# brontoguana/krasis

Measured on AMD Instinct MI355X. Metric: decode tok/s, Qwen3-Coder-Next Q4 @1 MI355X (KR_DECODE_FAST tolerance mode; both modes: value_exact / value_fast), higher is better.
Workload: dtype int4-g128 w x int16 act -> i32, f32 scales; 1 GPU; Qwen3-Coder-Next Q4 int4gpu on 1×MI355X (512-expert top-10, hybrid linear+GQA, FP8 KV); kv=FP8-E4M3 KV cache, kv_max_seq 256, layers=48, parallelism=one GPU holds the whole model (N > 1 lines: expert parallelism, see main_multi), hip_graph=True

## Files before the change

krasis_amd/csrc/kr_decode.cpp:

```cpp
#include <algorithm>
#include <hip/hip_runtime.h>

#include <cmath>
#include <cstring>
#include <memory>
#include <string>
#include <vector>

#include "../../include/krasis_hip.h"
#include "kr_decode_ops.h"
#include "kr_engine_internal.h"
#include "kr_kernels.h"
#include "kr_prefill.h"
#include "kr_router.h"
#include "kr_sampler.h"
#include <chrono>

#include "kr_decode_internal.h"
#include "kr_decode_fast.h"

static void prof_mark(kr_decode_store* s, int kind, hipStream_t st) {
    if (!s->prof) return;
    if (s->ev_used + 2 > s->ev_pool.size()) { for (int i = 0; i < 64; i++) { hipEvent_t e; (void)hipEventCreate(&e); s->ev_pool.push_back(e); } }
    if (kind >= 0) s->ev_kind.push_back(kind);
// ... 626 lines not shown
    PROF(PK_MATVEC, kr_launch_matvec(mv(s, L.mqb_wid), s->proj_b.p, 1, q_full, st));
}

static int attn_mla(StepCtx& cx, DLayer& L, size_t li) {
    kr_decode_store* s = cx.s; hipStream_t st = cx.st;
    if (!L.kv_k.p) return kr_fail(KR_ERR_STATE, "set_decode_state was not called (no MLA cache for layer %zu)", li);
    if (L.mla_rope_seq < s->kv_max_seq) return kr_fail(KR_ERR_VALUE, "MLA rope table (%d) shorter than kv_max_seq (%d)", L.mla_rope_seq, s->kv_max_seq);
    float* kv_out = (float*)s->kbuf.p; float* q_full = (float*)s->proj_a.p;
    const bool lora = L.mq_wid < 0;
    if (!cx.did_in) {
        const int wids[2] = {L.kva_wid, lora ? L.mqa_wid : L.mq_wid};
        float* ys[2] = {kv_out, lora ? (float*)s->proj_b.p : q_full};
        proj_group(cx, wids, ys, 2, cx.hid, 1);
    }
    if (lora) mla_lora_tail(cx, L, q_full);
    KrMlaArgs a{};
    a.step = (const KrStep*)s->step_dev.p; a.kv_out = kv_out; a.q_full = q_full; a.kv_a_norm = (const float*)L.kv_a_norm.p; a.w_kc = (const float*)L.w_kc.p;
    a.w_vc = (const float*)L.w_vc.p; a.rope_cos = (const float*)L.mla_cos.p; a.rope_sin = (const float*)L.mla_sin.p;
    a.ckv_cache = L.kv_k.p; a.kpe_cache = L.kv_v.p; a.kv_fp8 = s->kv_fp8; a.q_abs = (float*)s->qbuf.p; a.q_pe = (float*)s->zbuf.p;
    a.attn_lat = (float*)s->latbuf.p; a.v_proj = (float*)s->attn_out.p;
    a.nh = L.nh; a.klr = L.klr; a.nd = L.nd; a.rd = L.rd; a.vhd = L.vhd; a.eps = s->eps; a.sm_scale = L.sm_scale;
    a.sc_g = s->kv_max_seq > s->mla_split_min ? (float*)s->gqa_scores.p : nullptr;
    if (s->attn_fast && a.sc_g) { a.fast = 1; a.fd_o = (float*)s->fd_o.p; a.fd_ml = (float*)s->fd_ml.p; }
    a.decode_fast = cx.fast ? 1 : 0; a.decode_fused = cx.fast && s->opt_gqa_fused ? 1 : 0;
    PROF(PK_GQA, kr_launch_mla(a, s->kv_max_seq, st));
    if (cx.fast && s->weights[L.o_wid]->cols == L.nh * L.vhd) {
        KrFdmArgs fo = fdm_one(s, 2, L.o_wid, cx.hid); fo.hid_in = (const float*)s->attn_out.p;
        if (PROF_RC(PK_OUT_PROJ, kr_launch_fdm(fo, st)) == 0) return KR_OK;
    }
    out_proj(cx, L.o_wid, false);
    return KR_OK;
}

static int fast_moe(StepCtx& cx, DLayer& L, Layer& EL, size_t li, bool* done) {
    kr_decode_store* s = cx.s; kr_engine* e = cx.e; hipStream_t st = cx.st;
    if (EL.gguf && cx.src.mode == 2) return KR_OK;
    const MoeShape m = moe_shape(s, L, EL);
    KrFmoeArgs fa{}; KrMoeArgs& a = fa.m;
    moe_args_common(cx, L, m, a);
    a.act_img = s->img_post.p; a.act_img_bf16 = s->img_post_bf16.p;
    a.ids = (const int32_t*)s->r_ids.p; a.wts = (const float*)s->r_w.p;
    a.topk = s->topk; a.n_slots = m.n_slots; a.I = EL.inter; a.gu = (float*)s->moe_gu.p; a.eo = (float*)s->moe_eo.p;
    bool ok = true;
    if (EL.gguf) {
        fa.gguf = 1; fa.ggate = EL.g_gate.view(); fa.gup = EL.g_up.view(); fa.gdown = EL.g_down.view(); fa.act_f32 = (const float*)s->hid2.p;
        a.E = e->cfg.n_routed_experts; ok = e->r_ne == e->cfg.n_routed_experts;
    } else { a.E = e->r_ne; a.w13 = EL.w13.view(); a.w2 = EL.w2.view(); }
    if (m.has_gate) {
        const KrMatDev sg = mv(s, L.sg_wid);
        if (EL.gguf ? sg.bits == a.sw13.bits : (a.w13.bits == a.sw13.bits && sg.bits == a.w13.bits)) { a.sgate = sg; a.gate_out = (float*)s->gate_val.p; }
        else ok = false;
    }
    fa.logits = (const float*)s->r_logits.p; fa.esc = route_esc(EL); fa.scoring = s->scoring; fa.norm_topk = s->norm_topk;
    fa.hid_out = cx.hid;
    if (cx.ep_dec) {
        kr_ep_slice(e, &a.e_lo, &a.e_hi, &a.e_sub);
        fa.shared_skip = m.has_shared && kr_ep_rank(e) != (int)(li % (size_t)kr_ep_world(e)) ? 1 : 0;
    }
    if (!ok || kr_fmoe_check(fa) != 0) return KR_OK;
    if (PROF_RC(PK_ROUTE_LOGITS, kr_launch_frt(frt_args(cx, L, EL), st)) != 0) return KR_OK;
    const int r13 = PROF_RC(PK_MOE_W13, kr_launch_fw13(fa, st));
    const int r2 = PROF_RC(PK_MOE_W2, kr_launch_fw2(fa, st));
    if ((r13 || r2) && EL.gguf) return kr_fail(KR_ERR_STATE, "internal: KR_DECODE_FAST expert launch refused after kr_fmoe_check accepted GGUF layer %zu", li);
    if (r13 || r2) return kr_fail(KR_ERR_STATE, "internal: KR_DECODE_FAST expert launch refused after kr_fmoe_check accepted layer %zu", li);
    if (cx.ep_dec) if (int rc = kr_ep_allreduce_on(e, cx.hid, (size_t)cx.H, st)) return rc;
    cx.res_cur = cx.other(); cx.src = KrNormSrc{}; *done = true;
    return KR_OK;
}

static bool dense_fast(StepCtx& cx, DLayer& L) {
    kr_decode_store* s = cx.s; hipStream_t st = cx.st;
    const KrMatDev g = mv(s, L.gate_wid), u = mv(s, L.up_wid);
    const int K = s->weights[L.down_wid]->cols;
    if (!(g.bits == u.bits && (g.bits == 4 || g.bits == 8))) return false;
    KrFdmArgs fd = fdm_one(s, 1, L.gate_wid, (float*)s->dense_gu.p);
    fdm_norm(cx, L.post_norm, fd);
    fd.mm.n = 2; fd.mm.m[1] = u; fd.mm.y[1] = (float*)s->dense_gu.p + K; fd.mm.tile_end[1] = fd.mm.tile_end[0] + (u.N + 7) / 8;
    if (PROF_RC(PK_MATVEC, kr_launch_fdm(fd, st)) != 0) return false;
    cx.res_cur = cx.other();
    PROF(PK_MATVEC, kr_launch_matvec(mv(s, L.down_wid), s->dense_gu.p, 1, cx.hid, st, KR_ACT_SILU_MUL));
    return true;
}

static int moe_exact_gguf(StepCtx& cx, DLayer& L, Layer& EL, const float* act, bool routed) {
    kr_decode_store* s = cx.s; kr_engine* e = cx.e; hipStream_t st = cx.st;
    const MoeShape m = moe_shape(s, L, EL);
    const int k = s->topk, H = cx.H;
    GgMoeArgs g{};
    g.B = 1; g.topk = k; g.n_slots = k; g.H = H; g.E = e->cfg.n_routed_experts; g.act_f32 = act; g.ids = (const int32_t*)s->r_ids.p;
    g.gate = EL.g_gate.view(); g.up = EL.g_up.view(); g.down = EL.g_down.view();
    g.I_max = EL.inter; g.gu_ld = 2 * m.imax;
    g.gu = (float*)s->moe_gu.p; g.eo = (float*)s->moe_eo.p;
    PROF(PK_MOE_W13, kr_launch_gguf_moe(g, st));
    if (m.has_shared) {
        KrMoeArgs a{};
        moe_args_common(cx, L, m, a);
        a.act_f32 = act; if (routed && cx.img_ok()) { a.act_img = s->img_post.p; a.act_img_bf16 = s->img_post_bf16.p; }
        a.topk = 0; a.n_slots = 1; a.E = 0; a.I = m.I_shared;
        a.w13 = a.sw13; a.w2 = a.sw2;
        a.gu = g.gu + (size_t)k * g.gu_ld; a.eo = g.eo + (size_t)k * H;
        const bool fuse_gate = m.has_gate && mv(s, L.sg_wid).bits == a.sw13.bits;
        if (fuse_gate) { a.sgate = mv(s, L.sg_wid); a.gate_out = (float*)s->gate_val.p; }
        PROF(PK_MOE_W13, kr_launch_moe_w13(a, st));
        if (m.has_gate && !fuse_gate) PROF(PK_SHARED_GATE, kr_launch_matvec(mv(s, L.sg_wid), act, 1, (float*)s->gate_val.p, st));
        PROF(PK_MOE_W2, kr_launch_moe_w2(a, st));
    }
    if (cx.fast) {
// ... 159 lines not shown
    if (token == KR_TOKEN_FROM_DEVICE) kr_launch_set_step_dev((KrStep*)s->step_dev.p, (const int*)s->tok.p, pos, st);
    else kr_launch_set_step((KrStep*)s->step_dev.p, token, pos, st);
    s->last_stream = st;
    const bool ep_active = kr_ep_decode_active(s->eng);
    if (s->eng->ep_generation != s->ep_generation_seen) {
        s->ep_generation_seen = s->eng->ep_generation; s->graph_ok = false; s->ep_eager_steps = 0;
    }
    if (ep_active && s->ep_eager_steps < 2) s->ep_eager_steps++;
    else if (s->use_graph && (!ep_active || (s->opt_ep_graph && kr_ep_is_rccl(s->eng)))) {
        if (!s->graph_ok) {
            if (s->graph_exec) { (void)hipGraphExecDestroy(s->graph_exec); s->graph_exec = nullptr; }
            hipGraph_t g = nullptr;
            KR_HIP(hipStreamBeginCapture(st, hipStreamCaptureModeThreadLocal));
            const int rc = enqueue_step(s, st);
            hipError_t ce = hipStreamEndCapture(st, &g);
            if (rc) { if (g) (void)hipGraphDestroy(g); return rc; }
            if (ce != hipSuccess) return kr_fail(KR_ERR_HIP, "hipStreamEndCapture failed: %s", hipGetErrorString(ce));
            KR_HIP(hipGraphInstantiate(&s->graph_exec, g, nullptr, nullptr, 0));
            (void)hipGraphDestroy(g);
            s->graph_ok = true;
        }
        KR_HIP(hipGraphLaunch(s->graph_exec, st));
        return KR_OK;
    }
    return enqueue_step(s, st);
}

extern "C" int kr_decode_set_kv_dtype(kr_decode_store* s, int kv_dtype) {
    if (int rc = chk_store(s)) return rc;
    if (kv_dtype != 0 && kv_dtype != 1) return kr_fail(KR_ERR_VALUE, "kv_dtype %d unknown (0 = FP16, 1 = FP8-E4M3)", kv_dtype);
    if (s->kv_fp8 != kv_dtype) for (auto& L : s->layers) if (L.attn == ATTN_GQA || L.attn == ATTN_MLA) { L.kv_k.release(); L.kv_v.release(); }
    s->kv_fp8 = kv_dtype; s->graph_ok = false;
    return KR_OK;
}

extern "C" int kr_decode_set_attention_mode(kr_decode_store* s, int mode) {
    if (int rc = chk_store(s)) return rc;
    if (mode < 0 || mode > 7) return kr_fail(KR_ERR_VALUE, "numerics mode %d unknown (bit 0 = KR_ATTN_FAST, bit 1 = KR_GEMM_FAST, bit 2 = KR_DECODE_FAST)", mode);
    s->attn_fast = mode & 1; s->gemm_fast = (mode >> 1) & 1; s->decode_fast = (mode >> 2) & 1; s->graph_ok = false;
    return KR_OK;
}

extern "C" int kr_decode_set_option(kr_decode_store* s, const char* name, int value) {
    if (int rc = chk_store(s)) return rc;
    if (!name) return kr_fail(KR_ERR_VALUE, "null option name");
    if (!strcmp(name, "gqa_stream")) { s->opt_gqa_stream = value != 0; s->graph_ok = false; return KR_OK; }
    if (!strcmp(name, "w2_combine")) { s->opt_w2_combine = value != 0; s->graph_ok = false; return KR_OK; }
    if (!strcmp(name, "la_heads")) { s->opt_la_heads = value != 0; s->graph_ok = false; return KR_OK; }
    if (!strcmp(name, "lm_fused")) { s->opt_lm_fused = value != 0; s->graph_ok = false; return KR_OK; }
    if (!strcmp(name, "gqa_fused")) { s->opt_gqa_fused = value != 0; s->graph_ok = false; return KR_OK; }
    if (!strcmp(name, "gemm_ring")) { kr_pfr_set_enabled(value); return KR_OK; }
    if (!strcmp(name, "la_conv_fused")) { s->opt_la_conv_fused = value != 0; return KR_OK; }
    if (!strcmp(name, "dense_fast")) { s->opt_dense_fast = value != 0; s->graph_ok = false; return KR_OK; }
    if (!strcmp(name, "norm_rows")) { s->opt_norm_rows = value != 0; return KR_OK; }
    if (!strcmp(name, "pfm_timing")) { s->opt_pfm_timing = value != 0; return KR_OK; }
    if (!strcmp(name, "generate_lookahead")) { s->opt_gen_lookahead = value != 0; return KR_OK; }
    if (!strcmp(name, "multi_sample_loop")) { s->opt_multi_sample_loop = value != 0; return KR_OK; }
    if (!strcmp(name, "multi_attn_fast")) { s->opt_multi_attn_fast = value != 0; return KR_OK; }
    if (!strcmp(name, "multi_attn_fast_paged")) { s->opt_multi_attn_fast_paged = value != 0; return KR_OK; }
    if (!strcmp(name, "multi_mla_fast")) { s->opt_multi_mla_fast = value != 0; return KR_OK; }
    if (!strcmp(name, "multi_extend_la_chunk")) { s->opt_multi_extend_la_chunk = value != 0; return KR_OK; }
    if (!strcmp(name, "multi_extend_exact_mfma")) { s->opt_multi_extend_exact_mfma = value != 0; return KR_OK; }
    if (!strcmp(name, "multi_extend_mla_exact_mfma")) { s->opt_multi_extend_mla_exact_mfma = value != 0; return KR_OK; }
    if (!strcmp(name, "multi_attn_exact_split")) { s->opt_multi_attn_exact_split = value != 0; return KR_OK; }
    if (!strcmp(name, "multi_attn_exact_split_min")) {
        if (value < 1) return kr_fail(KR_ERR_VALUE, "multi_attn_exact_split_min %d: at least 1", value);
        s->opt_multi_attn_exact_split_min = value; return KR_OK;
    }
    if (!strcmp(name, "multi_mla_exact_split")) { s->opt_multi_mla_exact_split = value != 0; return KR_OK; }
    if (!strcmp(name, "multi_mla_exact_split_min")) {
        if (value < 1) return kr_fail(KR_ERR_VALUE, "multi_mla_exact_split_min %d: at least 1", value);
        s->opt_multi_mla_exact_split_min = value; return KR_OK;
    }
    if (!strcmp(name, "multi_extend_flash")) { s->opt_multi_extend_flash = value != 0; return KR_OK; }
    if (!strcmp(name, "multi_extend_mla_flash")) { s->opt_multi_extend_mla_flash = value != 0; return KR_OK; }
    if (!strcmp(name, "gguf_exact_pass")) { s->opt_gguf_exact_pass = value != 0; return KR_OK; }
    if (!strcmp(name, "gguf_exact_grouped")) { s->opt_gguf_exact_grouped = value != 0; return KR_OK; }
    if (!strcmp(name, "ep_graph")) { s->opt_ep_graph = value != 0; s->graph_ok = false; return KR_OK; }
    return kr_fail(KR_ERR_VALUE, "unknown option '%s'", name);
}

extern "C" int kr_decode_set_use_graph(kr_decode_store* s, int enable) {
    if (int rc = chk_store(s)) return rc;
    s->use_graph = enable != 0; return KR_OK;
}

static int decode_step_on(kr_decode_store* s, int token_id, int position, float* logits_out, hipStream_t st) {
    {
        kr_engine* e = s->eng; size_t gu = 0, eo = 0;
        for (auto& L : s->layers) if (L.mlp == MLP_MOE) {
            if (s->own_eng || L.moe_layer >= (int)e->layers.size()) return kr_fail(KR_ERR_STATE, "set_moe_store was not called (MoE layer %d has no engine)", L.moe_layer);
            const MoeShape m = moe_shape(s, L, e->layers[L.moe_layer]);
            gu = maxz(gu, (size_t)m.n_slots * 2 * m.imax * 4); eo = maxz(eo, (size_t)m.n_slots * s->hidden * 4);
        }
        if (gu && (gu > s->moe_gu.bytes || eo > s->moe_eo.bytes || (size_t)e->r_ne * 4 > s->r_logits.bytes)) s->graph_ok = false;
        if (gu && (s->moe_gu.ensure(gu) || s->moe_eo.ensure(eo) || s->r_logits.ensure((size_t)e->r_ne * 4) || s->r_ids.ensure(256) || s->r_w.ensure(256)))
            return kr_fail(KR_ERR_HIP, "hipMalloc failed");
    }
    if (int rc = run_step(s, token_id, position, st)) return rc;
    if (logits_out) {
        if (is_device_ptr(logits_out)) KR_HIP(hipMemcpyAsync(logits_out, s->logits.p, (size_t)s->vocab * 4, hipMemcpyDeviceToDevice, st));
        else { KR_HIP(hipMemcpyAsync(logits_out, s->logits.p, (size_t)s->vocab * 4, hipMemcpyDeviceToHost, st)); KR_HIP(hipStreamSynchronize(st)); }
    }
    return KR_OK;
}

// ... 200 lines not shown
```

krasis_amd/csrc/kr_decode_fast.h:

```cpp
#pragma once
#include <hip/hip_runtime.h>
#include <stdint.h>

#include "kr_decode_ops.h"
#include "kr_kernels.h"
#include "kr_gguf.h"

struct KrFdmArgs {
    KrMultiMat mm;
    int mode;
    const void* img;
    const float *hid_in, *res_in, *norm_w; float* res_out;
    const float* emb; const KrStep* step;
    int first; float eps; int bias_one;
    float* conv_state; const float* conv_w; float *qk_out, *v_out, *z_out; int nk, dk, hr, dv; int conv_mi, gate_mi;
    const float *a_log, *dt_bias; float *ge_out, *beta_out;
};
int kr_launch_fdm(const KrFdmArgs& a, hipStream_t st);

struct KrFlaArgs {
    const float *qk, *v, *z, *ge, *beta; float scale;
    float* state; const float* norm_w; float* out; void* img_out; int img_k;
    int nk, nv, hr, dk, dv; float eps;
};
int kr_launch_fla(const KrFlaArgs& a, hipStream_t st);

struct KrFrtArgs {
    const void* gate_cm; int gate_bf16; const float* bias; float* logits; int E, H;
    const float *hid_in, *res_in, *norm_w; float *hid_out, *res_out; float eps; int bias_one;
    void *img_f32, *img_bf16;
};
int kr_launch_frt(const KrFrtArgs& a, hipStream_t st);

struct KrFmoeArgs {
    KrMoeArgs m;
    const float* logits; const float* esc; int scoring, norm_topk;
    float* hid_out;
    int gguf;
    GgMat ggate, gup, gdown;
    const float* act_f32;
    int shared_skip;
};
int kr_fmoe_check(const KrFmoeArgs& a);
int kr_launch_fw13(const KrFmoeArgs& a, hipStream_t st);
int kr_launch_fw2(const KrFmoeArgs& a, hipStream_t st);

int kr_launch_fgqa(const KrGqaArgs& a, int max_seq, hipStream_t st);
int kr_launch_fmla(const KrMlaArgs& a, int max_seq, hipStream_t st);
```

krasis_amd/csrc/kr_decode_fast.hip:

```cpp
#include "kr_decode_fast.h"
#include "kr_gguf_dev.h"

#include "kr_device.h"
#include "kr_libm.h"
#include "kr_exact_dev.h"
#include "kr_matvec_dev.h"
#include "kr_topk.h"

typedef float f32x4 __attribute__((ext_vector_type(4)));
extern __shared__ __attribute__((aligned(16))) u32x4 kr_fsm[];

#ifdef KR_FTIMING
__device__ unsigned long long kr_fstamps[8][16];
#define KR_FSTAMP(k, i) do { if (blockIdx.x == gridDim.x / 2 && blockIdx.y == 0 && threadIdx.x == 0) kr_fstamps[k][i] = wall_clock64(); } while (0)
extern "C" int kr_debug_fstamps(unsigned long long* out) { return (int)hipMemcpyFromSymbol(out, HIP_SYMBOL(kr_fstamps), sizeof(kr_fstamps)); }
__device__ unsigned long long kr_fwg[6][1024][3];
#define KR_FWG(k, i) do { if (threadIdx.x == 0) { const unsigned b_ = blockIdx.x + gridDim.x * blockIdx.y; if (b_ < 1024) { kr_fwg[k][b_][i] = wall_clock64(); \
        if ((i) == 0) kr_fwg[k][b_][2] = (unsigned long long)__builtin_amdgcn_s_getreg((4 << 0) | (0 << 6) | (31 << 11)) | ((unsigned long long)__builtin_amdgcn_s_getreg((20 << 0) | (0 << 6) | (3 << 11)) << 32); } } } while (0)
extern "C" int kr_debug_fwg(unsigned long long* out) { return (int)hipMemcpyFromSymbol(out, HIP_SYMBOL(kr_fwg), sizeof(kr_fwg)); }
#else
#define KR_FSTAMP(k, i) do { } while (0)
#define KR_FWG(k, i) do { } while (0)
#endif

#define KR_FW2_LDS_MAX (64 * 1024)
#define KR_FU 16

__device__ __forceinline__ float kr_f_red8(float v) {
    v += __int_as_float(KR_DPP(__float_as_int(v), KR_DPP_XOR1));
    v += __int_as_float(KR_DPP(__float_as_int(v), KR_DPP_XOR2));
    v += __int_as_float(KR_DPP(__float_as_int(v), KR_DPP_HALF_MIRROR));
    return v;
}
__device__ __forceinline__ float kr_f_red16(float v) {
    v = kr_f_red8(v);
    v += __int_as_float(KR_DPP(__float_as_int(v), KR_DPP_MIRROR));
    return v;
}
__device__ __forceinline__ float kr_f_rl(float v, int l) { return __int_as_float(__builtin_amdgcn_readlane(__float_as_int(v), l)); }
__device__ __forceinline__ float kr_f_wave_sum(float v) {
    v = kr_f_red16(v);
    return (kr_f_rl(v, 0) + kr_f_rl(v, 16)) + (kr_f_rl(v, 32) + kr_f_rl(v, 48));
}
__device__ __forceinline__ float kr_f_wave_max(float v) {
    v = kr_red16_max_f32(v);
    return fmaxf(fmaxf(kr_f_rl(v, 0), kr_f_rl(v, 16)), fmaxf(kr_f_rl(v, 32), kr_f_rl(v, 48)));
}
__device__ __forceinline__ void kr_f_wave_sync() { __builtin_amdgcn_fence(__ATOMIC_ACQ_REL, "workgroup"); __builtin_amdgcn_wave_barrier(); }

template <int BITS, int NU, int FU = KR_FU> struct KrFw { u32x4 w[NU > 0 ? NU : FU]; uint32_t sc[NU > 0 ? NU : FU]; };

template <int BITS, int NU, int FU = KR_FU>
__device__ __forceinline__ void kr_f_fetch(KrFw<BITS, NU, FU>& p, const KrMatDev& m, const void* qbase, const uint32_t* sbase, int tile, int lane, int ub, int u1) {
    const int units = BITS == 4 ? m.ngp : m.ng;
    const u32x4* q = reinterpret_cast<const u32x4*>(qbase) + (size_t)tile * units * 64 + lane;
    const uint32_t* s = sbase + (size_t)tile * m.ngp * 8 + (lane >> 3);
    if constexpr (NU > 0) {
#pragma unroll
        for (int u = 0; u < NU; u++) { p.w[u] = kr_ldg_nt(q + (size_t)(ub + u) * 64); p.sc[u] = kr_ldg_nt(s + (BITS == 4 ? (ub + u) : ((ub + u) >> 1)) * 8); }
    } else {
#pragma unroll
        for (int u = 0; u < FU; u++)
            if (ub + u < u1) { p.w[u] = kr_ldg_nt(q + (size_t)(ub + u) * 64); p.sc[u] = kr_ldg_nt(s + (BITS == 4 ? (ub + u) : ((ub + u) >> 1)) * 8); }
    }
}

template <int BITS, int NU, int FU = KR_FU>
__device__ __forceinline__ float kr_f_dot(const KrFw<BITS, NU, FU>& p, const KrMatDev& m, int ub, int u1, int l8, const KrActLds& L, float acc) {
    constexpr int N = NU > 0 ? NU : FU;
#pragma unroll
    for (int u = 0; u < N; u++) {
        const int un = ub + u;
        if (NU > 0 || un < u1) {
            if constexpr (BITS == 4) {
// ... 520 lines not shown
    }
    if (raw) {
#pragma unroll
        for (int i = 0; i < NV; i++) sc[i] = lg[i];
    } else if (scoring == 0) {
        const int e8 = (E / 8) * 8;
#pragma unroll
        for (int i = 0; i < NV; i++) { const int e = lane * NV + i; sc[i] = e < E ? (e < e8 ? kr_sigmoid_poly4(lg[i]) : 1.0f / (1.0f + kr_expf(-lg[i]))) : 0.0f; }
    } else {
        float mx = lg[0];
#pragma unroll
        for (int i = 1; i < NV; i++) mx = fmaxf(mx, lg[i]);
        mx = kr_f_wave_max(mx);
        float se = 0.0f;
#pragma unroll
        for (int i = 0; i < NV; i++) { const int e = lane * NV + i; sc[i] = e < E ? __builtin_amdgcn_exp2f((lg[i] - mx) * 1.4426950408889634f) : 0.0f; se += sc[i]; }
        se = kr_f_wave_sum(se);
        const float inv = 1.0f / se;
#pragma unroll
        for (int i = 0; i < NV; i++) sc[i] *= inv;
    }
    const bool on_logits = scoring == 1 && esc == nullptr;
#pragma unroll
    for (int i = 0; i < NV; i++) {
        const int e = lane * NV + i;
        sl[i] = on_logits ? lg[i] : ((!raw && esc && e < E) ? sc[i] + esc[e] : sc[i]);
        if (e < E) { scores[e] = sc[i]; sel[e] = sl[i]; }
    }
    const int np = k + 1 <= E ? k + 1 : k;
    if (!kr_f_topk<NV>(sl, E, np, pv, pi, cand)) kr_topk_wave_reg<NV>(sl, E, np, pv, pi);
    kr_f_wave_sync();
    {
        const float pa = lane < np ? pv[lane] : 0.0f, pb = lane + 1 < np ? pv[lane + 1] : 0.0f;
        const bool tie = __ballot(lane + 1 < np && pa == pb) != 0ull;
        if (tie) {
            if (lane == 0) kr_topk_heap_serial(sel, E, k, hv, hi, pi);
            kr_f_wave_sync();
        }
    }
    const int my = lane < k ? pi[lane] : 0;
    float wv = lane < k ? scores[my] : 0.0f;
    if (raw) {
        const float mx = kr_f_wave_max(lane < k ? wv : -__builtin_inff());
        wv = lane < k ? kr_expf(wv - mx) : 0.0f;
    }
    if (raw || norm) {
        const float se = kr_f_wave_sum(wv);
        if (raw) wv = wv * (1.0f / se);
        else if (se > 0.0f) wv = wv / se;
    }
    if (lane < k) { s_ids[lane] = my; s_w[lane] = wv; }
}

template <int BITS, int NU>
__global__ void __launch_bounds__(256) kr_fw13_kernel(const float* p_logits, const float* p_esc, const void* p_img_bf16, int p_E, int p_topk, int p_scoring, int p_norm, int p_H, int p_I, int p_gguf,
                                                      const KrFmoeArgs fa) {
    const KrMoeArgs& a = fa.m;
    constexpr int KS = 2, TW = 2;
    __shared__ int s_ids[32];
    __shared__ float s_w[32];
    __shared__ float s_x[TW][KS][2][8];
    const int slot = blockIdx.y;
    const bool shared = slot >= p_topk;
    if (!shared && (int)blockIdx.x * 2  >= p_I / 8) return;
    const int t = threadIdx.x, wave = t >> 6, lane = t & 63, l8 = lane & 7, cl = lane >> 3;
    const int tw = wave >> 1, ks = wave & 1;
    const KrActLds L = kr_carve_lds(kr_fsm, p_H, BITS == 8);
    const bool gg = p_gguf && !shared;
    const GgAct GA = gg_carve(reinterpret_cast<char*>(kr_fsm), p_H);
    const size_t img_bytes = p_gguf ? (kr_lds_bytes(p_H, BITS == 8) > gg_lds_bytes(p_H, false) ? kr_lds_bytes(p_H, BITS == 8) : gg_lds_bytes(p_H, false)) : kr_lds_bytes(p_H, BITS == 8);
    KR_FSTAMP(4, 0); KR_FWG(4, 0);
    if (shared) kr_f_image_copy<BITS>(a.act_img, p_H, kr_fsm, L, t, 256);
    else if (wave > 0) {
        if (gg) {
            for (int c = t - 64; c < a.H / 8; c += 192) {
                float v[8];
                kr_load8(fa.act_f32, c, v);
#pragma unroll
                for (int i = 0; i < 8; i++) v[i] = kr_bf16_to_f32(kr_f32_to_bf16(v[i]));
                gg_quant_store(v, c, GA);
            }
        } else kr_f_image_copy<BITS>(p_img_bf16, p_H, kr_fsm, L, t - 64, 192);
    } else {
        float* selsm = reinterpret_cast<float*>(reinterpret_cast<char*>(kr_fsm) + img_bytes);
        const int nv = (p_E + 63) / 64;
        if (nv <= 1) kr_f_select<1>(p_logits, p_esc, p_E, p_topk, p_scoring, p_norm, selsm, s_ids, s_w);
        else if (nv <= 2) kr_f_select<2>(p_logits, p_esc, p_E, p_topk, p_scoring, p_norm, selsm, s_ids, s_w);
        else if (nv <= 4) kr_f_select<4>(p_logits, p_esc, p_E, p_topk, p_scoring, p_norm, selsm, s_ids, s_w);
        else kr_f_select<8>(p_logits, p_esc, p_E, p_topk, p_scoring, p_norm, selsm, s_ids, s_w);
        if (blockIdx.x == 0 && slot == 0 && lane < p_topk) {
            const_cast<int32_t*>(a.ids)[lane] = s_ids[lane]; const_cast<float*>(a.wts)[lane] = s_w[lane];
        }
    }
    KR_FSTAMP(4, 1);
    __syncthreads();
    KR_FSTAMP(4, 2);
    if (gg) {
        int e = s_ids[slot];
        if (a.e_hi > 0) { if (e < a.e_lo || e >= a.e_hi) return; e -= a.e_sub; }
        const GgMat gm = gg_expert_mat(fa.ggate, e), um = gg_expert_mat(fa.gup, e);
        const int ntp = gm.N / 8, unit = blockIdx.x * TW + tw;
        float ag = 0.0f, au = 0.0f;
        if (unit < ntp) {
            if (gm.type == GG_Q4_K) ag = gg_tile_q4k(gm, unit, GA, lane, ks, KS); else if (gm.type == GG_Q8_0) ag = gg_tile_q8_0(gm, unit, GA, lane, ks, KS); else ag = gg_tile_q4_0(gm, unit, GA, lane, ks, KS);
            if (um.type == GG_Q4_K) au = gg_tile_q4k(um, unit, GA, lane, ks, KS); else if (um.type == GG_Q8_0) au = gg_tile_q8_0(um, unit, GA, lane, ks, KS); else au = gg_tile_q4_0(um, unit, GA, lane, ks, KS);
        }
        if (l8 == 0) { s_x[tw][ks][0][cl] = ag; s_x[tw][ks][1][cl] = au; }
        __syncthreads();
        if (ks == 0 && l8 == 0 && unit < ntp) {
            const float g = s_x[tw][0][0][cl] + s_x[tw][1][0][cl], u = s_x[tw][0][1][cl] + s_x[tw][1][1][cl];
            a.gu[(size_t)slot * a.gu_ld + unit * 8 + cl] = (g / (1.0f + kr_expf(-g))) * u;
        }
        return;
    }
    const KrMatDev& m = shared ? a.sw13 : a.w13;
    const void* qb = m.q; const uint32_t* sb = m.s;
    const int inter = shared ? a.I_shared : a.I;
    if (!shared) {
        int e = s_ids[slot];
        if (a.e_hi > 0) {
            if (e < a.e_lo || e >= a.e_hi) return;
            e -= a.e_sub;
        }
        qb = reinterpret_cast<const char*>(m.q) + (size_t)e * m.q_stride;
        sb = reinterpret_cast<const uint32_t*>(reinterpret_cast<const char*>(m.s) + (size_t)e * m.s_stride);
    } else if (fa.shared_skip) return;
    const int ntp = inter / 8;
    const int unit = blockIdx.x * TW + tw;
    const bool pair = unit < ntp;
    const bool gate_row = shared && a.sgate.q != nullptr && unit == ntp;
    const int units = BITS == 4 ? m.ngp : m.ng;
    int u0, u1;
    if (NU > 0) { u0 = ks * NU; u1 = u0 + NU; }
    else { const int uw = (units + KS - 1) / KS; u0 = ks * uw; u1 = u0 + uw < units ? u0 + uw : units; }
    KrFw<BITS, NU, 8> Wg, Wu;
    float ag = 0.0f, au = 0.0f;
    if (pair) {
        kr_f_fetch<BITS, NU, 8>(Wg, m, qb, sb, unit, lane, u0, u1);
        kr_f_fetch<BITS, NU, 8>(Wu, m, qb, sb, unit + ntp, lane, u0, u1);
        KR_FSTAMP(4, 3);
        ag = kr_f_tile<BITS, NU, 8>(Wg, m, qb, sb, unit, lane, u0, u1, L);
        au = kr_f_tile<BITS, NU, 8>(Wu, m, qb, sb, unit + ntp, lane, u0, u1, L);
    } else if (gate_row) {
        kr_f_fetch<BITS, NU, 8>(Wg, a.sgate, a.sgate.q, a.sgate.s, 0, lane, u0, u1);
        ag = kr_f_tile<BITS, NU, 8>(Wg, a.sgate, a.sgate.q, a.sgate.s, 0, lane, u0, u1, L);
    }
    KR_FSTAMP(4, 4);
    if (l8 == 0) { s_x[tw][ks][0][cl] = ag; s_x[tw][ks][1][cl] = au; }
    __syncthreads();
    if (ks == 0 && l8 == 0) {
        const float g = s_x[tw][0][0][cl] + s_x[tw][1][0][cl], u = s_x[tw][0][1][cl] + s_x[tw][1][1][cl];
        if (pair) a.gu[(size_t)slot * a.gu_ld + unit * 8 + cl] = (g * kr_sigmoid_poly5(g)) * u;
        else if (gate_row && cl == 0) a.gate_out[0] = 1.0f / (1.0f + kr_expf(-g));
    }
    KR_FSTAMP(4, 5); KR_FWG(4, 1);
}

template <int BITS, int NU, bool MULTI>
__global__ void __launch_bounds__(1024) kr_fw2_kernel(const float* p_gu, const int32_t* p_ids, const float* p_wts, int p_gu_ld, int p_topk, int slot_lds, int pr_, int ps_, const KrFmoeArgs fa) {
    const KrMoeArgs& a = fa.m;
    const int pr = MULTI ? pr_ : 1, ps = MULTI ? ps_ : 1;
    __shared__ float s_y[16][8];
    __shared__ __attribute__((aligned(16))) float s_wt[16];
    const int t = threadIdx.x, vslot = t >> 6, lane = t & 63, l8 = lane & 7, cl = lane >> 3;
    const int nrw = p_topk * pr;
    const int slot = vslot < nrw ? vslot / pr : p_topk, part = vslot < nrw ? vslot % pr : vslot - nrw, parts = vslot < nrw ? pr : ps;
    const int tile = blockIdx.x;
    KR_FSTAMP(5, 0); KR_FWG(5, 0);
    const float sig = (a.gate_out && !fa.shared_skip) ? a.gate_out[0] : 1.0f;
    const bool shared = slot >= p_topk;
    const bool gg = fa.gguf && !shared;
    const KrMatDev& m = (shared || fa.gguf) ? a.sw2 : a.w2;
    const int inter = shared ? a.I_shared : a.I;
    constexpr int HCN = (NU > 0 && !MULTI) ? (BITS == 4 ? NU / 2 : NU / 4) : 0;
    constexpr int HC = HCN > 0 ? 1 : 0;
    const int units = BITS == 4 ? m.ngp : m.ng;
    const int u0 = units * part / parts, u1 = units * (part + 1) / parts;
    const int cpu = (BITS == 4 ? 256 : 128) / 8;
    const int c0 = u0 * cpu + lane, cend = u1 * cpu < inter / 8 ? u1 * cpu : inter / 8;
    constexpr bool PRE = !MULTI;
    [[maybe_unused]] float hpre[1][8];
    if constexpr (PRE) kr_load8(p_gu + (size_t)slot * p_gu_ld, c0 < inter / 8 ? c0 : inter / 8 - 1, hpre[0]);
    const void* qb = m.q; const uint32_t* sb = m.s;
    bool valid = true; float wt = 1.0f;
    bool skip = false;
    size_t ee = 0;
    if (!shared) {
        int e = p_ids[slot];
        valid = e >= 0 && e < a.E; wt = p_wts[slot];
        if (a.e_hi > 0) { skip = !valid || e < a.e_lo || e >= a.e_hi; e -= a.e_sub; }
        ee = valid && !skip ? (size_t)e : 0;
        if (!gg) {
            qb = reinterpret_cast<const char*>(m.q) + ee * m.q_stride;
// ... 461 lines not shown
    if (a.H % 128 || a.H > 4096 || a.H < 256) return 1;
    const size_t lds = (size_t)16 * (a.H / 16 + 4) * 4;
    dim3 grid((a.E + 3) / 4);
    const int ncg = a.gate_bf16 ? a.H / 128 : a.H / 64, cpw = (ncg + 3) / 4;
#define KR_FRT(B_, C_) hipLaunchKernelGGL((kr_frt_kernel<B_, C_>), grid, dim3(256), lds, st, a.hid_in, a.res_in, a.norm_w, a.gate_cm, a.H, a)
    if (a.gate_bf16) { if (cpw <= 1) KR_FRT(true, 1); else if (cpw <= 2) KR_FRT(true, 2); else if (cpw <= 4) KR_FRT(true, 4); else KR_FRT(true, 8); }
    else { if (cpw <= 2) KR_FRT(false, 2); else if (cpw <= 4) KR_FRT(false, 4); else if (cpw <= 8) KR_FRT(false, 8); else KR_FRT(false, 16); }
#undef KR_FRT
    return 0;
}

static bool kr_fmoe_ok(const KrFmoeArgs& fa) {
    const KrMoeArgs& a = fa.m;
    const bool has_shared = a.n_slots > a.topk;
    if (a.B != 1 || a.n_slots > 16 || a.topk > 15 || a.E > 512 || a.act_mode != KR_ACT_SILU_FUSED) return false;
    if (fa.gguf) {
        auto ok_mat = [&](const GgMat& g, int K, int N) { return (g.type == GG_Q4_K ? K % 256 == 0 : ((g.type == GG_Q8_0 || g.type == GG_Q4_0) && K % 32 == 0)) && g.K == K && g.N == N && N % 8 == 0; };
        if (!fa.act_f32 || !ok_mat(fa.ggate, a.H, a.I) || !ok_mat(fa.gup, a.H, a.I) || !ok_mat(fa.gdown, a.I, a.H) || a.H % 128) return false;
        if (has_shared) {
            if (!a.act_img || a.sw13.bits != a.sw2.bits || a.I_shared % 128 || a.sw13.ng * 128 != a.H || a.sw2.ng * 128 != a.I_shared) return false;
            if (a.sgate.q && (a.sgate.bits != a.sw13.bits || a.sgate.ng != a.sw13.ng || !a.gate_out)) return false;
        }
        return true;
    }
    if (!a.act_img || !a.act_img_bf16 || a.H % 128 || a.I % 128) return false;
    if (a.w13.ng * 128 != a.H || a.w2.ng * 128 != a.I) return false;
    if (has_shared) {
        if (a.sw13.bits != a.w13.bits || a.sw2.bits != a.w2.bits || a.I_shared % 128 || a.sw13.ng != a.w13.ng || a.sw2.ng * 128 != a.I_shared) return false;
        if (a.sgate.q && (a.sgate.bits != a.w13.bits || a.sgate.ng != a.w13.ng || !a.gate_out)) return false;
    }
    return true;
}

static size_t kr_fw2_slot_lds(const KrFmoeArgs& fa) {
    const KrMoeArgs& a = fa.m;
    const bool has_shared = a.n_slots > a.topk;
    const int imax = has_shared && a.I_shared > a.I ? a.I_shared : a.I;
    size_t n = fa.gguf ? (has_shared ? kr_lds_bytes(a.I_shared, a.sw2.bits == 8) : 0) : kr_lds_bytes(imax, a.w2.bits == 8);
    if (fa.gguf) { const size_t g = (gg_lds_bytes(a.I, false) + 15) & ~(size_t)15; if (g > n) n = g; }
    return n;
}
int kr_fmoe_check(const KrFmoeArgs& fa) {
    if (!kr_fmoe_ok(fa)) return 1;
    const KrMoeArgs& a = fa.m;
    return kr_fw2_slot_lds(fa) * a.n_slots > KR_FW2_LDS_MAX ? 1 : 0;
}

int kr_launch_fw13(const KrFmoeArgs& fa, hipStream_t st) {
    if (!kr_fmoe_ok(fa)) return 1;
    const KrMoeArgs& a = fa.m;
    const bool has_shared = a.n_slots > a.topk;
    int ntp = a.I / 8;
    if (has_shared && a.I_shared / 8 + (a.sgate.q ? 1 : 0) > ntp) ntp = a.I_shared / 8 + (a.sgate.q ? 1 : 0);
    dim3 grid((ntp + 1) / 2, a.n_slots);
    const KrMatDev& wm = fa.gguf ? a.sw13 : a.w13;
    const int wbits = fa.gguf && !has_shared ? 4 : wm.bits;
    size_t img = kr_lds_bytes(a.H, wbits == 8);
    if (fa.gguf && gg_lds_bytes(a.H, false) > img) img = gg_lds_bytes(a.H, false);
    const size_t lds = img + (size_t)(2 * a.E + 33 + 33 + 32 + 32 + 4 + 136) * 4;
    const int units = fa.gguf && !has_shared ? 0 : (wbits == 4 ? wm.ngp : wm.ng);
    const bool even = !fa.gguf && (a.w13.bits == 8 || (a.w13.ng % 2) == 0) && units % 2 == 0;
    const int nu = even ? units / 2 : 0;
#define KR_FW13(B_, N_) hipLaunchKernelGGL((kr_fw13_kernel<B_, N_>), grid, dim3(256), lds, st, fa.logits, fa.esc, a.act_img_bf16, a.E, a.topk, fa.scoring, fa.norm_topk, a.H, a.I, fa.gguf, fa)
    if (wbits == 4) { if (nu == 4) KR_FW13(4, 4); else if (nu == 8) KR_FW13(4, 8); else KR_FW13(4, 0); }
    else { if (nu == 8) KR_FW13(8, 8); else KR_FW13(8, 0); }
#undef KR_FW13
    return 0;
}

int kr_launch_fw2(const KrFmoeArgs& fa, hipStream_t st) {
    if (!kr_fmoe_ok(fa)) return 1;
    const KrMoeArgs& a = fa.m;
    const bool has_shared = a.n_slots > a.topk;
    const size_t slot_lds = kr_fw2_slot_lds(fa);
    if (slot_lds * a.n_slots > KR_FW2_LDS_MAX) return 1;
    dim3 grid((a.H + 7) / 8);
    const int wbits = fa.gguf ? (has_shared ? a.sw2.bits : 4) : a.w2.bits;
    const int units = fa.gguf ? 0 : (a.w2.bits == 4 ? a.w2.ngp : a.w2.ng);
    const bool uniform = !fa.gguf && (!has_shared || a.I_shared == a.I) && (a.w2.bits == 8 || a.w2.ng % 2 == 0);
    const int nu = uniform && (units == 2 || units == 4 || units == 6 || units == 8) ? units : 0;
    const int sunits = has_shared ? (a.sw2.bits == 4 ? a.sw2.ngp : a.sw2.ng) : 0;
    int pr = 1, ps = has_shared ? 1 : 0;
    if (nu == 0 && !fa.gguf && units >= 4 && a.I >= 1024 && a.topk <= 7) pr = 2;
    if (has_shared && nu == 0 && !fa.shared_skip) {
        ps = (a.I_shared * pr + a.I - 1) / a.I;
        if (ps > 4) ps = 4;
        while (ps > 1 && (a.topk * pr + ps > 16 || ps > sunits)) ps--;
    }
    const bool multi = pr > 1 || ps > 1;
#define KR_FW2(B_, N_, M_) hipLaunchKernelGGL((kr_fw2_kernel<B_, N_, M_>), grid, dim3(64 * (a.topk * pr + ps)), slot_lds * a.n_slots, st, a.gu, a.ids, a.wts, a.gu_ld, a.topk, (int)slot_lds, pr, ps, fa)
    if (multi) { if (wbits == 4) KR_FW2(4, 0, true); else KR_FW2(8, 0, true); }
    else if (wbits == 4) { if (nu == 2) KR_FW2(4, 2, false); else if (nu == 4) KR_FW2(4, 4, false); else if (nu == 6) KR_FW2(4, 6, false); else if (nu == 8) KR_FW2(4, 8, false); else KR_FW2(4, 0, false); }
    else { if (nu == 4) KR_FW2(8, 4, false); else if (nu == 8) KR_FW2(8, 8, false); else KR_FW2(8, 0, false); }
#undef KR_FW2
    return 0;
}
```

krasis_amd/csrc/kr_decode_internal.h:

```cpp
#pragma once
#include <hip/hip_runtime.h>

#include <memory>
#include <vector>

#include "kr_decode_ops.h"
#include "kr_engine_internal.h"
#include "kr_multi.h"
#include "kr_page_pool.h"
#include "kr_spec.h"

struct DWeight { MatSet ms; int rows = 0, cols = 0; };

enum { ATTN_NONE = 0, ATTN_LA = 1, ATTN_GQA = 2, ATTN_MLA = 3 };
enum { MLP_NONE = 0, MLP_MOE = 1, MLP_DENSE = 2 };

struct DLayer {
    int input_norm = -1, post_norm = -1;
    int attn = ATTN_NONE, mlp = MLP_NONE;
    int qkvz_wid = -1, ba_wid = -1, out_wid = -1, nk = 0, nv = 0, dk = 0, dv = 0, kd = 4; float la_scale = 1.0f;
    DevBuf conv_w, a_log, dt_bias, la_norm_w, conv_state, recur_state;
    int q_wid = -1, k_wid = -1, v_wid = -1, o_wid = -1, gated = 0, nh = 0, nkv = 0, hd = 0; float sm_scale = 1.0f;
    DevBuf q_norm, k_norm, kv_k, kv_v; int q_norm_len = 0, k_norm_len = 0;
    int kva_wid = -1, mq_wid = -1, mqa_wid = -1, mqb_wid = -1, klr = 0, nd = 0, rd = 0, vhd = 0, q_a_norm_len = 0;
    DevBuf w_kc, w_vc, kv_a_norm, q_a_norm, mla_cos, mla_sin; int mla_rope_seq = 0;
    int moe_layer = -1, sgu_wid = -1, sd_wid = -1, sg_wid = -1;
    int gate_wid = -1, up_wid = -1, down_wid = -1;
};

struct kr_multi_state {
    int n_slots = 0, max_seq = 0, kv_fp8 = 0;
    std::vector<DevBuf> a, b;
    std::vector<size_t> a_stride, b_stride;
    std::vector<size_t> a_row, b_row;
    KrPagePool pg; DevBuf pg_table, pg_pools, pg_new; int pg_npools = 0;
    DevBuf la_pools, fk_ids; int la_npools = 0;
    DevBuf rows, ids, logits, scores, scratch;
    DevBuf fd_o, fd_ml; bool fd_ready = false;
    DevBuf tiles;
    bool pf_ready = false, mf_ready = false, lc_ready = false;
    DevBuf lc_scratch;
    DevBuf xm_rows;
    bool mla_fd_ready = false;
    struct Sampler { float temperature = 0.0f, top_p = 1.0f, penalty = 0.0f; int top_k = 0; };
    std::vector<Sampler> smp; size_t smp_words = 0;
    DevBuf smp_seen, smp_rng;
    DevBuf smp_rows, smp_work, smp_sorted, smp_keys, smp_temp, smp_probs; size_t smp_temp_bytes = 0;
    DevBuf smp_hyp;
    DevBuf v_rec, v_tab, v_out, v_keep; std::vector<KrMultiLaCommit> v_host; std::vector<int> v_la_of;
    bool v_pending = false, v_sampled = false, v_has64 = false, v_has128 = false; int v_nv_max = 0, v_dv_max = 0; size_t v_rows = 0;
    std::vector<int32_t> v_match; hipStream_t v_st = nullptr;
    hipEvent_t ev = nullptr;
    ~kr_multi_state() { if (ev) (void)hipEventDestroy(ev); }
};

struct kr_standalone_state;
struct kr_decode_store {
    kr_standalone_state* standalone = nullptr;
    kr_engine* eng = nullptr; int device = 0; bool own_eng = false;
    int group_size = 128; bool norm_bias_one = false;
    std::vector<std::unique_ptr<DWeight>> weights;
    std::vector<std::unique_ptr<DevBuf>> norms; std::vector<int> norm_len;
    bool configured = false;
    int hidden = 0, n_layers = 0, vocab = 0, topk = 0, scoring = 1, norm_topk = 1, final_norm = -1, lm_head = -1;
    float eps = 1e-6f, rsf = 1.0f;
    DevBuf embedding;
    std::vector<DLayer> layers;
    DevBuf rope_cos, rope_sin; int rope_half = 0, max_rope_seq = 0;
    int kv_max_seq = 0;
    DevBuf hid, res, proj_a, proj_b, qbuf, kbuf, vbuf, zbuf, gbuf, betabuf, gatebuf, latbuf, recur_out, attn_out, logits, gate_val, tok;
    DevBuf dense_gu;
    DevBuf hid2, res2, r_counter, argmax_scratch;
    int kv_fp8 = 0;
    DevBuf img_in, img_post, img_post_bf16, img_attn;
    int opt_gqa_stream = 0, opt_pfm_timing = 0, opt_norm_rows = 1, opt_la_conv_fused = 1, opt_gqa_fused = 1, opt_lm_fused = 1, opt_la_heads = 1, opt_w2_combine = 1, opt_dense_fast = 1;
    int opt_multi_sample_loop = 0;
    int opt_gguf_exact_pass = 0;
    int opt_gguf_exact_grouped = 1;
    int opt_multi_attn_fast_paged = 0;
    int opt_multi_attn_fast = 0;
    int opt_multi_mla_fast = 0;
    int opt_multi_extend_flash = 0;
    int opt_multi_extend_la_chunk = 0;
    int opt_multi_attn_exact_split = 0;
    int opt_multi_attn_exact_split_min = 512;
    int opt_multi_mla_exact_split = 0;
    int opt_multi_mla_exact_split_min = 512;
    int opt_multi_extend_exact_mfma = 0;
    int opt_multi_extend_mla_exact_mfma = 0;
    int opt_multi_extend_mla_flash = 0;
    int opt_gen_lookahead = 0;
    int opt_ep_graph = 0;
    uint64_t ep_generation_seen = 0;
    int ep_eager_steps = 0;
    int* gen_ring = nullptr; int gen_ring_n = 0; hipEvent_t gen_ev[2] = {nullptr, nullptr};
    int decode_fast = 0; DevBuf f_qk;
    int gemm_fast = 0;
    int attn_fast = 0; DevBuf fd_o, fd_ml;
    DevBuf gqa_scores; int gqa_split_min = 1024, mla_split_min = 512;
    DevBuf smp_seen, smp_keys, smp_temp, smp_probs, smp_rng; size_t smp_temp_bytes = 0;
    DevBuf pf_scores;
    DevBuf pf_vlogits, pf_nll;
    DevBuf pf_tokens; int pf_chunk = 0; int pf_depth = 0; std::vector<hipStream_t> pf_side; std::vector<hipEvent_t> pf_events;
    DevBuf pf_scratch;
    DevBuf moe_gu, moe_eo, r_logits, r_ids, r_w;
    DevBuf step_dev; hipStream_t last_stream = nullptr;
    size_t weight_bytes = 0;
    std::vector<int> spec_la, spec_la_of; std::vector<KrSpecLa> spec_host; DevBuf spec_buf, spec_tab, spec_logits, spec_out, spec_part;
    std::unique_ptr<kr_multi_state> multi;
    bool spec_pending = false; int spec_n = 0, spec_match = 0, spec_nv_max = 0, spec_dv_max = 0; bool spec_has64 = false, spec_has128 = false; size_t spec_floats = 0; hipStream_t spec_st = nullptr;
    hipGraphExec_t graph_exec = nullptr; bool graph_ok = false; bool use_graph = true;
    bool prof = false; std::vector<hipEvent_t> ev_pool; size_t ev_used = 0; std::vector<int> ev_kind;
};

enum { PK_EMBED = 0, PK_RMSNORM, PK_MATVEC, PK_LA_CONV, PK_LA_RECUR, PK_GATED_NORM, PK_GQA, PK_ROUTE_LOGITS, PK_ROUTE_SELECT, PK_MOE_W13,
       PK_MOE_W2, PK_MOE_COMBINE, PK_LM_HEAD, PK_ARGMAX, PK_SHARED_GATE, PK_OUT_PROJ , PK_COUNT };


static inline KrMatDev mv(kr_decode_store* s, int wid) { return s->weights[wid]->ms.view(); }
int kr_ensure_wsum(kr_engine* e, MatSet& ms, hipStream_t st);
int kr_moe_prefill_prepare(kr_engine* e, int layer, int fast, int routed_only, hipStream_t st, int gguf_exact = 0);
void kr_standalone_release(kr_decode_store* s);
int kr_exact_refuse(kr_decode_store* s, bool slots);
int kr_spec_refuse(kr_decode_store* s);
bool paged_refused(const kr_decode_store* s);
bool has_attn(const kr_decode_store* s, int kind);
int kr_xm_refuse(kr_decode_store* s);
int kr_xs_refuse(kr_decode_store* s);
// ... 8 lines not shown
```

Baseline: 621.8 tok/s.

## Compute per-slot expert id in fused W13 instead of full top-k select

Each routed slot block's wave 0 now finds only its own expert rank with a register sorting network and wave-wide max rounds, rather than running the full top-k selection with weights in every block. One extra publishing block runs the full select and writes ids and weights for the W2 stage. If a tie or an invalid key is detected, the block falls back to the full select. The intent is to shorten the selection prologue that sits before weight fetch in every block, at the cost of an extra grid row and more complex control flow. It is enabled by default only for softmax scoring with normalised top-k, no expert bias and at most 512 experts.

```diff
diff --git a/krasis_amd/csrc/kr_decode.cpp b/krasis_amd/csrc/kr_decode.cpp
--- a/krasis_amd/csrc/kr_decode.cpp
+++ b/krasis_amd/csrc/kr_decode.cpp
@@ -702,7 +702,7 @@
         else ok = false;
     }
     fa.logits = (const float*)s->r_logits.p; fa.esc = route_esc(EL); fa.scoring = s->scoring; fa.norm_topk = s->norm_topk;
-    fa.hid_out = cx.hid;
+    fa.hid_out = cx.hid; fa.slot_select = s->opt_slot_select;
     if (cx.ep_dec) {
         kr_ep_slice(e, &a.e_lo, &a.e_hi, &a.e_sub);
         fa.shared_skip = m.has_shared && kr_ep_rank(e) != (int)(li % (size_t)kr_ep_world(e)) ? 1 : 0;
@@ -968,6 +968,7 @@
     if (!strcmp(name, "gemm_ring")) { kr_pfr_set_enabled(value); return KR_OK; }
     if (!strcmp(name, "la_conv_fused")) { s->opt_la_conv_fused = value != 0; return KR_OK; }
     if (!strcmp(name, "dense_fast")) { s->opt_dense_fast = value != 0; s->graph_ok = false; return KR_OK; }
+    if (!strcmp(name, "slot_select")) { s->opt_slot_select = value != 0; s->graph_ok = false; return KR_OK; }
     if (!strcmp(name, "norm_rows")) { s->opt_norm_rows = value != 0; return KR_OK; }
     if (!strcmp(name, "pfm_timing")) { s->opt_pfm_timing = value != 0; return KR_OK; }
     if (!strcmp(name, "generate_lookahead")) { s->opt_gen_lookahead = value != 0; return KR_OK; }
diff --git a/krasis_amd/csrc/kr_decode_fast.h b/krasis_amd/csrc/kr_decode_fast.h
--- a/krasis_amd/csrc/kr_decode_fast.h
+++ b/krasis_amd/csrc/kr_decode_fast.h
@@ -40,6 +40,7 @@
     GgMat ggate, gup, gdown;
     const float* act_f32;
     int shared_skip;
+    int slot_select;
 };
 int kr_fmoe_check(const KrFmoeArgs& a);
 int kr_launch_fw13(const KrFmoeArgs& a, hipStream_t st);
diff --git a/krasis_amd/csrc/kr_decode_fast.hip b/krasis_amd/csrc/kr_decode_fast.hip
--- a/krasis_amd/csrc/kr_decode_fast.hip
+++ b/krasis_amd/csrc/kr_decode_fast.hip
@@ -13,6 +13,7 @@
 #ifdef KR_FTIMING
 __device__ unsigned long long kr_fstamps[8][16];
 #define KR_FSTAMP(k, i) do { if (blockIdx.x == gridDim.x / 2 && blockIdx.y == 0 && threadIdx.x == 0) kr_fstamps[k][i] = wall_clock64(); } while (0)
+#define KR_FSTAMPY(k, i, row_) do { if (blockIdx.x == gridDim.x / 2 && (int)blockIdx.y == (row_) && threadIdx.x == 0) kr_fstamps[k][i] = wall_clock64(); } while (0)
 extern "C" int kr_debug_fstamps(unsigned long long* out) { return (int)hipMemcpyFromSymbol(out, HIP_SYMBOL(kr_fstamps), sizeof(kr_fstamps)); }
 __device__ unsigned long long kr_fwg[6][1024][3];
 #define KR_FWG(k, i) do { if (threadIdx.x == 0) { const unsigned b_ = blockIdx.x + gridDim.x * blockIdx.y; if (b_ < 1024) { kr_fwg[k][b_][i] = wall_clock64(); \
@@ -20,6 +21,7 @@
 extern "C" int kr_debug_fwg(unsigned long long* out) { return (int)hipMemcpyFromSymbol(out, HIP_SYMBOL(kr_fwg), sizeof(kr_fwg)); }
 #else
 #define KR_FSTAMP(k, i) do { } while (0)
+#define KR_FSTAMPY(k, i, y) do { } while (0)
 #define KR_FWG(k, i) do { } while (0)
 #endif
 
@@ -646,8 +648,84 @@
     if (lane < k) { s_ids[lane] = my; s_w[lane] = wv; }
 }
 
+__device__ __forceinline__ uint32_t kr_umin(uint32_t a, uint32_t b) { return a < b ? a : b; }
+#define KR_F_CEX(a_, b_) do { const uint32_t hi_ = kr_umax(s[a_], s[b_]), lo_ = kr_umin(s[a_], s[b_]); s[a_] = hi_; s[b_] = lo_; } while (0)
+template <int NV>
+__device__ __forceinline__ void kr_f_sort_desc(uint32_t (&s)[NV]) {
+    static_assert(NV == 1 || NV == 2 || NV == 4 || NV == 8, "networks for 1, 2, 4 and 8 keys");
+    if constexpr (NV == 2) { KR_F_CEX(0, 1); }
+    if constexpr (NV == 4) { KR_F_CEX(0, 2); KR_F_CEX(1, 3); KR_F_CEX(0, 1); KR_F_CEX(2, 3); KR_F_CEX(1, 2); }
+    if constexpr (NV == 8) {
+        KR_F_CEX(0, 2); KR_F_CEX(1, 3); KR_F_CEX(4, 6); KR_F_CEX(5, 7);
+        KR_F_CEX(0, 4); KR_F_CEX(1, 5); KR_F_CEX(2, 6); KR_F_CEX(3, 7);
+        KR_F_CEX(0, 1); KR_F_CEX(2, 3); KR_F_CEX(4, 5); KR_F_CEX(6, 7);
+        KR_F_CEX(2, 4); KR_F_CEX(3, 5);
+        KR_F_CEX(1, 4); KR_F_CEX(3, 6);
+        KR_F_CEX(1, 2); KR_F_CEX(3, 4); KR_F_CEX(5, 6);
+    }
+}
+#undef KR_F_CEX
+#define KR_FSEL(i) do { if (slot == 0) KR_FSTAMPY(7, (i), 0); else if (slot == k - 1) KR_FSTAMPY(7, 8 + (i), slot); } while (0)
+template <int NV>
+__device__ __forceinline__ bool kr_f_slot_select(const float* logits, int E, int k, int slot, int* s_id) {
+    const int lane = threadIdx.x & 63;
+    KR_FSEL(0);
+    float lg[NV];
+    if (NV % 4 == 0 && E % 4 == 0) {
+#pragma unroll
+        for (int i = 0; i + 3 < NV; i += 4) {
+            const int e = lane * NV + i;
+            const float4 v = *reinterpret_cast<const float4*>(logits + (e < E ? e : 0));
+            lg[i] = v.x; lg[i + 1] = v.y; lg[i + 2] = v.z; lg[i + 3] = v.w;
+        }
+    } else {
+#pragma unroll
+        for (int i = 0; i < NV; i++) { const int e = lane * NV + i; lg[i] = logits[e < E ? e : 0]; }
+    }
+#ifdef KR_FTIMING
+    asm volatile("s_waitcnt vmcnt(0)" ::: "memory");
+#endif
+    KR_FSEL(1);
+    uint32_t key[NV], s[NV];
+#pragma unroll
+    for (int i = 0; i < NV; i++) { const int e = lane * NV + i; key[i] = e < E ? kr_make_key(lg[i]) : 0u; s[i] = key[i]; }
+    kr_f_sort_desc<NV>(s);
+    KR_FSEL(2);
+    const int np = k + 1 <= E ? k + 1 : k;
+    const int rounds = slot + 2 < np ? slot + 2 : np;
+    uint32_t prev = 0u, vs = 0u;
+    int win_s = 0;
+    bool tie = false;
+    for (int r = 0; r < rounds; r++) {
+        const uint32_t w = kr_wave_umax(s[0]);
+        const uint64_t mask = __ballot(s[0] == w);
+        const int win = __builtin_ctzll(mask);
+        if (r == slot) {
+            vs = w; win_s = win;
+            tie = (mask & (mask - 1ull)) != 0ull || (r > 0 && prev == w);
+            if constexpr (NV > 1) tie = tie || (uint32_t)__builtin_amdgcn_readlane((int)s[1], win) == w;
+        } else if (r > slot) tie = tie || w == vs;
+        if (lane == win) {
+#pragma unroll
+            for (int i = 0; i + 1 < NV; i++) s[i] = s[i + 1];
+            s[NV - 1] = 0u;
+        }
+        prev = w;
+    }
+    KR_FSEL(3);
+    if (tie || vs == 0u) return false;
+    if (lane == win_s) {
+        int idx = 0;
+#pragma unroll
+        for (int i = NV - 1; i >= 0; i--) if (key[i] == vs) idx = i;
+        *s_id = lane * NV + idx;
+    }
+    KR_FSEL(4);
+    return true;
+}
+
 template <int BITS, int NU>
-__global__ void __launch_bounds__(256) kr_fw13_kernel(const float* p_logits, const float* p_esc, const void* p_img_bf16, int p_E, int p_topk, int p_scoring, int p_norm, int p_H, int p_I, int p_gguf,
+__global__ void __launch_bounds__(256) kr_fw13_kernel(const float* p_logits, const float* p_esc, const void* p_img_bf16, int p_E, int p_topk, int p_scoring, int p_norm, int p_H, int p_I, int p_gguf, int p_pub,
                                                       const KrFmoeArgs fa) {
     const KrMoeArgs& a = fa.m;
     constexpr int KS = 2, TW = 2;
@@ -655,15 +733,17 @@
     __shared__ float s_w[32];
     __shared__ float s_x[TW][KS][2][8];
     const int slot = blockIdx.y;
-    const bool shared = slot >= p_topk;
-    if (!shared && (int)blockIdx.x * 2  >= p_I / 8) return;
+    const bool pub = p_pub != 0 && slot == p_pub;
+    if (pub && (blockIdx.x != 0 || threadIdx.x >= 64)) return;
+    const bool shared = slot >= p_topk && !pub;
+    if (slot < p_topk && (int)blockIdx.x * 2  >= p_I / 8) return;
     const int t = threadIdx.x, wave = t >> 6, lane = t & 63, l8 = lane & 7, cl = lane >> 3;
     const int tw = wave >> 1, ks = wave & 1;
     const KrActLds L = kr_carve_lds(kr_fsm, p_H, BITS == 8);
     const bool gg = p_gguf && !shared;
     const GgAct GA = gg_carve(reinterpret_cast<char*>(kr_fsm), p_H);
     const size_t img_bytes = p_gguf ? (kr_lds_bytes(p_H, BITS == 8) > gg_lds_bytes(p_H, false) ? kr_lds_bytes(p_H, BITS == 8) : gg_lds_bytes(p_H, false)) : kr_lds_bytes(p_H, BITS == 8);
-    KR_FSTAMP(4, 0); KR_FWG(4, 0);
+    KR_FSTAMP(4, 0); KR_FWG(4, 0); KR_FSTAMPY(7, 13, p_topk - 1);
     if (shared) kr_f_image_copy<BITS>(a.act_img, p_H, kr_fsm, L, t, 256);
     else if (wave > 0) {
         if (gg) {
@@ -678,14 +758,24 @@
     } else {
         float* selsm = reinterpret_cast<float*>(reinterpret_cast<char*>(kr_fsm) + img_bytes);
         const int nv = (p_E + 63) / 64;
-        if (nv <= 1) kr_f_select<1>(p_logits, p_esc, p_E, p_topk, p_scoring, p_norm, selsm, s_ids, s_w);
-        else if (nv <= 2) kr_f_select<2>(p_logits, p_esc, p_E, p_topk, p_scoring, p_norm, selsm, s_ids, s_w);
-        else if (nv <= 4) kr_f_select<4>(p_logits, p_esc, p_E, p_topk, p_scoring, p_norm, selsm, s_ids, s_w);
-        else kr_f_select<8>(p_logits, p_esc, p_E, p_topk, p_scoring, p_norm, selsm, s_ids, s_w);
-        if (blockIdx.x == 0 && slot == 0 && lane < p_topk) {
-            const_cast<int32_t*>(a.ids)[lane] = s_ids[lane]; const_cast<float*>(a.wts)[lane] = s_w[lane];
-        }
-    }
+        bool full = true;
+        if (p_pub != 0 && !pub) {
+            if (nv <= 1) full = !kr_f_slot_select<1>(p_logits, p_E, p_topk, slot, &s_ids[slot]);
+            else if (nv <= 2) full = !kr_f_slot_select<2>(p_logits, p_E, p_topk, slot, &s_ids[slot]);
+            else if (nv <= 4) full = !kr_f_slot_select<4>(p_logits, p_E, p_topk, slot, &s_ids[slot]);
+            else full = !kr_f_slot_select<8>(p_logits, p_E, p_topk, slot, &s_ids[slot]);
+        }
+        if (full) {
+            if (nv <= 1) kr_f_select<1>(p_logits, p_esc, p_E, p_topk, p_scoring, p_norm, selsm, s_ids, s_w);
+            else if (nv <= 2) kr_f_select<2>(p_logits, p_esc, p_E, p_topk, p_scoring, p_norm, selsm, s_ids, s_w);
+            else if (nv <= 4) kr_f_select<4>(p_logits, p_esc, p_E, p_topk, p_scoring, p_norm, selsm, s_ids, s_w);
+            else kr_f_select<8>(p_logits, p_esc, p_E, p_topk, p_scoring, p_norm, selsm, s_ids, s_w);
+            if ((p_pub != 0 ? pub : (blockIdx.x == 0 && slot == 0)) && lane < p_topk) {
+                const_cast<int32_t*>(a.ids)[lane] = s_ids[lane]; const_cast<float*>(a.wts)[lane] = s_w[lane];
+            }
+        }
+    }
+    if (pub) return;
     KR_FSTAMP(4, 1);
     __syncthreads();
     KR_FSTAMP(4, 2);
@@ -732,7 +822,7 @@
     if (pair) {
         kr_f_fetch<BITS, NU, 8>(Wg, m, qb, sb, unit, lane, u0, u1);
         kr_f_fetch<BITS, NU, 8>(Wu, m, qb, sb, unit + ntp, lane, u0, u1);
-        KR_FSTAMP(4, 3);
+        KR_FSTAMP(4, 3); KR_FSTAMPY(7, 14, p_topk - 1);
         ag = kr_f_tile<BITS, NU, 8>(Wg, m, qb, sb, unit, lane, u0, u1, L);
         au = kr_f_tile<BITS, NU, 8>(Wu, m, qb, sb, unit + ntp, lane, u0, u1, L);
     } else if (gate_row) {
@@ -1300,7 +1390,9 @@
     const bool has_shared = a.n_slots > a.topk;
     int ntp = a.I / 8;
     if (has_shared && a.I_shared / 8 + (a.sgate.q ? 1 : 0) > ntp) ntp = a.I_shared / 8 + (a.sgate.q ? 1 : 0);
-    dim3 grid((ntp + 1) / 2, a.n_slots);
+    const bool per_slot = fa.slot_select != 0 && fa.scoring == 1 && fa.esc == nullptr && fa.norm_topk != 0 && a.E <= 512 && a.topk + 1 <= 64;
+    const int pub = per_slot ? a.n_slots : 0;
+    dim3 grid((ntp + 1) / 2, a.n_slots + (per_slot ? 1 : 0));
     const KrMatDev& wm = fa.gguf ? a.sw13 : a.w13;
     const int wbits = fa.gguf && !has_shared ? 4 : wm.bits;
     size_t img = kr_lds_bytes(a.H, wbits == 8);
@@ -1309,7 +1401,7 @@
     const int units = fa.gguf && !has_shared ? 0 : (wbits == 4 ? wm.ngp : wm.ng);
     const bool even = !fa.gguf && (a.w13.bits == 8 || (a.w13.ng % 2) == 0) && units % 2 == 0;
     const int nu = even ? units / 2 : 0;
-#define KR_FW13(B_, N_) hipLaunchKernelGGL((kr_fw13_kernel<B_, N_>), grid, dim3(256), lds, st, fa.logits, fa.esc, a.act_img_bf16, a.E, a.topk, fa.scoring, fa.norm_topk, a.H, a.I, fa.gguf, fa)
+#define KR_FW13(B_, N_) hipLaunchKernelGGL((kr_fw13_kernel<B_, N_>), grid, dim3(256), lds, st, fa.logits, fa.esc, a.act_img_bf16, a.E, a.topk, fa.scoring, fa.norm_topk, a.H, a.I, fa.gguf, pub, fa)
     if (wbits == 4) { if (nu == 4) KR_FW13(4, 4); else if (nu == 8) KR_FW13(4, 8); else KR_FW13(4, 0); }
     else { if (nu == 8) KR_FW13(8, 8); else KR_FW13(8, 0); }
 #undef KR_FW13
diff --git a/krasis_amd/csrc/kr_decode_internal.h b/krasis_amd/csrc/kr_decode_internal.h
--- a/krasis_amd/csrc/kr_decode_internal.h
+++ b/krasis_amd/csrc/kr_decode_internal.h
@@ -73,7 +73,7 @@
     DevBuf hid2, res2, r_counter, argmax_scratch;
     int kv_fp8 = 0;
     DevBuf img_in, img_post, img_post_bf16, img_attn;
-    int opt_gqa_stream = 0, opt_pfm_timing = 0, opt_norm_rows = 1, opt_la_conv_fused = 1, opt_gqa_fused = 1, opt_lm_fused = 1, opt_la_heads = 1, opt_w2_combine = 1, opt_dense_fast = 1;
+    int opt_gqa_stream = 0, opt_pfm_timing = 0, opt_norm_rows = 1, opt_la_conv_fused = 1, opt_gqa_fused = 1, opt_lm_fused = 1, opt_la_heads = 1, opt_w2_combine = 1, opt_dense_fast = 1, opt_slot_select = 1;
     int opt_multi_sample_loop = 0;
     int opt_gguf_exact_pass = 0;
     int opt_gguf_exact_grouped = 1;
```

Measured after the change: 633.9 tok/s (median of 6 runs). +1.9%, better.
